# tulip-control/polytope

Hardware: AMD Instinct MI355X
Metric: LP solves/sec (batched Chebyshev + redundancy) (higher is better)
Workload: dtype f64

## Files before the change

polytope_amd/csrc/plp_lane_lp.hpp:

```cpp
#pragma once
#include <math.h>

#if defined(__HIPCC__)
#include "plp_common.hpp"
#define PLP_LANE_FN __device__ __forceinline__
#else
#define PLP_LANE_FN static inline
namespace plp {
enum : int { ST_OPT = 0, ST_ITER = 1, ST_INFEAS = 2, ST_UNBND = 3, ST_NUM = 4 };
constexpr int ST_RETRY = 5;
constexpr double TOL_D = 1e-9, TOL_PIV = 1e-7, DEGEN_EPS = 1e-12;
constexpr int BLAND_AFTER = 6;
}
#endif

namespace plp {
namespace lane {

constexpr int LANE_MAX_ITERS = 48;
constexpr double LANE_TOL_D = 1e-11, LANE_TOL_PIV = 1e-11;
constexpr double LANE_M_NOISE = 64 * 2.220446049250313e-16;

struct Lp3 {
    double x0, x1, x2;
    int w0, w1, w2;
    int nact;
    int status;
    int iters;
    int ndeg;
};

PLP_LANE_FN void cross3(double a0, double a1, double a2, double b0, double b1, double b2, double& e0, double& e1,
                        double& e2) {
    e0 = fma(a1, b2, -(a2 * b1));
    e1 = fma(a2, b0, -(a0 * b2));
    e2 = fma(a0, b1, -(a1 * b0));
}

PLP_LANE_FN double dot3(double a0, double a1, double a2, double b0, double b1, double b2) {
    return fma(a2, b2, fma(a1, b1, a0 * b0));
}

template <class AnyF>
PLP_LANE_FN void proj1(const double c0, const double c1, const double c2, const double cn1, const double n0, const double n1,
                       const double n2, const double nn, double& d0, double& d1, double& d2, double& scale, AnyF ANY) {
    const double cn = dot3(c0, c1, c2, n0, n1, n2);
    d0 = fma(cn, n0, -(nn * c0));
    d1 = fma(cn, n1, -(nn * c1));
    d2 = fma(cn, n2, -(nn * c2));
    scale = nn;
    const double pn1 = fabs(d0) + fabs(d1) + fabs(d2);
    const bool small = (pn1 > 0.0) & (pn1 < 1e-4 * (nn * cn1));
    if (ANY(small)) {
        const double np_ = dot3(n0, n1, n2, d0, d1, d2);
        const double q0 = fma(nn, d0, -(np_ * n0)), q1 = fma(nn, d1, -(np_ * n1)), q2 = fma(nn, d2, -(np_ * n2));
        d0 = small ? q0 : d0;
        d1 = small ? q1 : d1;
        d2 = small ? q2 : d2;
        scale = small ? nn * nn : nn;
    }
}

constexpr double LANE_PAIR_SIN2 = 1e-10;

template <class RowF, class RatioF, class Ratio0F, class AnyF>
PLP_LANE_FN void walk3(Lp3& S, const double c0, const double c1, const double c2, const bool go, RowF ROWS, RatioF RATIO,
                       Ratio0F RATIO0, AnyF ANY, const bool warm = false) {
    if (!warm) {
        S.x0 = S.x1 = S.x2 = 0.0;
        S.w0 = S.w1 = S.w2 = -1;
        S.nact = 0;
        S.iters = 0;
        S.ndeg = 0;
    }
    S.status = go ? -1 : ST_OPT;
    const double cn1 = fabs(c0) + fabs(c1) + fabs(c2);
    if (go && !(cn1 > 0.0)) S.status = ST_OPT;
    if (!warm && ANY(S.status < 0)) {
        const bool step = S.status < 0;
        const double d0 = -c0, d1 = -c1, d2 = -c2;
        const double tolp = LANE_TOL_PIV * cn1;
        double bs = 1.0, bd = 0.0;
        int bi = -1;
        RATIO0(d0, d1, d2, tolp, bs, bd, bi);
        if (step) {
            S.iters = 1;
            if (bi < 0) {
                S.status = ST_UNBND;
            } else {
                const double t = bs / bd;
                S.x0 = fma(t, d0, 0.0);
                S.x1 = fma(t, d1, 0.0);
                S.x2 = fma(t, d2, 0.0);
                S.w0 = bi;
                S.nact = 1;
                S.ndeg = (t * cn1 <= DEGEN_EPS) ? 1 : 0;
            }
        }
    }
    while (ANY(S.status < 0)) {
        const bool run = S.status < 0;
        double d0 = -c0, d1 = -c1, d2 = -c2;
        double n00 = 0, n01 = 0, n02 = 0, n10 = 0, n11 = 0, n12 = 0, n20 = 0, n21 = 0, n22 = 0;
        if (ANY(run && S.nact >= 1)) {
            if (S.nact >= 1) ROWS(S.w0, n00, n01, n02);
            if (S.nact >= 2) ROWS(S.w1, n10, n11, n12);
            if (S.nact >= 3) ROWS(S.w2, n20, n21, n22);
        }
        bool stalled = false;
        double dscale = cn1;
        if (S.nact == 1) {
            const double nn = dot3(n00, n01, n02, n00, n01, n02);
            double sc;
            proj1(c0, c1, c2, cn1, n00, n01, n02, nn, d0, d1, d2, sc, ANY);
            dscale = sc * cn1;
        } else if (S.nact == 2) {
            double e0, e1, e2;
            cross3(n00, n01, n02, n10, n11, n12, e0, e1, e2);
            const double ce = dot3(c0, c1, c2, e0, e1, e2);
            d0 = -(ce * e0);
            d1 = -(ce * e1);
            d2 = -(ce * e2);
            dscale = dot3(e0, e1, e2, e0, e1, e2) * cn1;
            const double nn0 = dot3(n00, n01, n02, n00, n01, n02), nn1 = dot3(n10, n11, n12, n10, n11, n12);
            if (run && !(dot3(e0, e1, e2, e0, e1, e2) > LANE_PAIR_SIN2 * nn0 * nn1)) S.status = ST_RETRY;
        } else if (S.nact == 3) {
            d0 = d1 = d2 = 0.0;
        }
        {
            const double dn1 = fabs(d0) + fabs(d1) + fabs(d2);
            stalled = !(dn1 > LANE_TOL_D * dscale);
        }
        if (ANY(S.status < 0 && stalled)) {
            if (S.status < 0 && stalled) {
                if (S.nact == 0) {
                    S.status = ST_OPT;
                } else if (S.nact == 1) {
                    const double cn = dot3(c0, c1, c2, n00, n01, n02);
                    if (cn <= 0.0) S.status = ST_OPT;
                    else { S.nact = 0; d0 = -c0; d1 = -c1; d2 = -c2; }
                } else if (S.nact == 2) {
                    const double g00 = dot3(n00, n01, n02, n00, n01, n02), g11 = dot3(n10, n11, n12, n10, n11, n12);
                    const double g01 = dot3(n00, n01, n02, n10, n11, n12);
                    const double r0 = -dot3(c0, c1, c2, n00, n01, n02), r1 = -dot3(c0, c1, c2, n10, n11, n12);
                    const double l0 = fma(r0, g11, -(r1 * g01)), l1 = fma(r1, g00, -(r0 * g01));
                    const double w0 = 0.5 * (1.0 + g00), w1 = 0.5 * (1.0 + g11);
                    const double tol0 = LANE_TOL_D * g11 * w0 * cn1, tol1 = LANE_TOL_D * g00 * w1 * cn1;
                    if (l0 >= -tol0 && l1 >= -tol1) S.status = ST_OPT;
                    else {
                        const bool drop0 = l0 * w0 < l1 * w1;
                        if (drop0) { S.w0 = S.w1; n00 = n10; n01 = n11; n02 = n12; }
                        S.nact = 1;
                        double sc;
                        proj1(c0, c1, c2, cn1, n00, n01, n02, dot3(n00, n01, n02, n00, n01, n02), d0, d1, d2, sc, [](bool q) { return q; });
                    }
                } else {
                    double u00, u01, u02, u10, u11, u12, u20, u21, u22;
                    cross3(n10, n11, n12, n20, n21, n22, u00, u01, u02);
                    cross3(n20, n21, n22, n00, n01, n02, u10, u11, u12);
                    cross3(n00, n01, n02, n10, n11, n12, u20, u21, u22);
                    const double det = dot3(n00, n01, n02, u00, u01, u02);
                    const double g00 = dot3(n00, n01, n02, n00, n01, n02), g11 = dot3(n10, n11, n12, n10, n11, n12);
                    const double g22 = dot3(n20, n21, n22, n20, n21, n22);
                    if (!(det * det > 1e-18 * (g00 * g11 * g22))) {
                        S.status = ST_RETRY;
                    } else {
                        const double sg = det > 0.0 ? 1.0 : -1.0;
                        const double l0 = -sg * dot3(c0, c1, c2, u00, u01, u02);
                        const double l1 = -sg * dot3(c0, c1, c2, u10, u11, u12);
                        const double l2 = -sg * dot3(c0, c1, c2, u20, u21, u22);
                        const double a0 = l0 * (0.5 * (1.0 + g00)), a1 = l1 * (0.5 * (1.0 + g11)), a2 = l2 * (0.5 * (1.0 + g22));
                        const double tol = LANE_TOL_D * fabs(det) * cn1;
                        if (a0 >= -tol && a1 >= -tol && a2 >= -tol) S.status = ST_OPT;
                        else {
                            int j = 0;
                            double am = a0;
                            if (a1 < am) { am = a1; j = 1; }
                            if (a2 < am) { am = a2; j = 2; }
                            double gg;
                            if (j == 0) { d0 = -sg * u00; d1 = -sg * u01; d2 = -sg * u02; S.w0 = S.w1; S.w1 = S.w2; gg = g11 * g22; }
                            else if (j == 1) { d0 = -sg * u10; d1 = -sg * u11; d2 = -sg * u12; S.w1 = S.w2; gg = g22 * g00; }
                            else { d0 = -sg * u20; d1 = -sg * u21; d2 = -sg * u22; gg = g00 * g11; }
                            S.nact = 2;
                            if (!(dot3(d0, d1, d2, d0, d1, d2) > LANE_PAIR_SIN2 * gg)) S.status = ST_RETRY;
                        }
                    }
                }
            }
        }
        const bool step = S.status < 0;
        const double dn1 = fabs(d0) + fabs(d1) + fabs(d2);
        const double tolp = LANE_TOL_PIV * dn1;
        double bs = 1.0, bd = 0.0;
        int bi = -1;
        if (ANY(step)) RATIO(d0, d1, d2, S.x0, S.x1, S.x2, tolp, bs, bd, bi);
        if (step) {
            ++S.iters;
            if (bi < 0) {
                S.status = ST_UNBND;
            } else {
                const double t = bs / bd;
                S.x0 = fma(t, d0, S.x0);
                S.x1 = fma(t, d1, S.x1);
                S.x2 = fma(t, d2, S.x2);
                if (S.nact == 0) S.w0 = bi;
                else if (S.nact == 1) S.w1 = bi;
                else S.w2 = bi;
                S.nact += 1;
                S.ndeg = (t * dn1 <= DEGEN_EPS) ? S.ndeg + 1 : 0;
                if (S.ndeg >= BLAND_AFTER || S.iters >= LANE_MAX_ITERS) S.status = ST_RETRY;
            }
        }
    }
}

template <class RowF, class RatioF, class AnyF>
PLP_LANE_FN void walk3(Lp3& S, const double c0, const double c1, const double c2, const bool go, RowF ROWS, RatioF RATIO,
                       AnyF ANY, const bool warm = false) {
    walk3(S, c0, c1, c2, go, ROWS, RATIO,
          [&](double d0, double d1, double d2, double tolp, double& bs, double& bd, int& bi) {
              RATIO(d0, d1, d2, 0.0, 0.0, 0.0, tolp, bs, bd, bi);
          },
          ANY, warm);
}

struct Lp4 {
    double x0, x1, x2, x3;
    int w0, w1, w2, w3;
    int nact, status, iters, ndeg;
};

PLP_LANE_FN double dot4(double a0, double a1, double a2, double a3, double b0, double b1, double b2, double b3) {
    return fma(a3, b3, fma(a2, b2, fma(a1, b1, a0 * b0)));
}

PLP_LANE_FN void gcross4(double p0, double p1, double p2, double p3, double q0, double q1, double q2, double q3, double r0,
                         double r1, double r2, double r3, double& e0, double& e1, double& e2, double& e3) {
    const double m01 = fma(q0, r1, -(q1 * r0)), m02 = fma(q0, r2, -(q2 * r0)), m03 = fma(q0, r3, -(q3 * r0));
    const double m12 = fma(q1, r2, -(q2 * r1)), m13 = fma(q1, r3, -(q3 * r1)), m23 = fma(q2, r3, -(q3 * r2));
    e0 = fma(p1, m23, fma(-p2, m13, p3 * m12));
    e1 = -fma(p0, m23, fma(-p2, m03, p3 * m02));
    e2 = fma(p0, m13, fma(-p1, m03, p3 * m01));
    e3 = -fma(p0, m12, fma(-p1, m02, p2 * m01));
}

template <class RowF, class RatioF, class AnyF>
PLP_LANE_FN void walk4(Lp4& S, const double c0, const double c1, const double c2, const double c3, const bool go, RowF ROWS,
                       RatioF RATIO, AnyF ANY) {
    S.x0 = S.x1 = S.x2 = S.x3 = 0.0;
    S.w0 = S.w1 = S.w2 = S.w3 = -1;
    S.nact = 0;
    S.iters = 0;
    S.ndeg = 0;
    S.status = go ? -1 : ST_OPT;
    const double cn1 = fabs(c0) + fabs(c1) + fabs(c2) + fabs(c3);
    if (go && !(cn1 > 0.0)) S.status = ST_OPT;
    while (ANY(S.status < 0)) {
        const bool run = S.status < 0;
        bool dropped = false;
        double d0 = -c0, d1 = -c1, d2 = -c2, d3 = -c3;
        double n00 = 0, n01 = 0, n02 = 0, n03 = 0, n10 = 0, n11 = 0, n12 = 0, n13 = 0;
        double n20 = 0, n21 = 0, n22 = 0, n23 = 0, n30 = 0, n31 = 0, n32 = 0, n33 = 0;
        if (ANY(run && S.nact >= 1)) {
            if (S.nact >= 1) ROWS(S.w0, n00, n01, n02, n03);
            if (S.nact >= 2) ROWS(S.w1, n10, n11, n12, n13);
            if (S.nact >= 3) ROWS(S.w2, n20, n21, n22, n23);
            if (S.nact >= 4) ROWS(S.w3, n30, n31, n32, n33);
        }
        const double g00 = dot4(n00, n01, n02, n03, n00, n01, n02, n03), g11 = dot4(n10, n11, n12, n13, n10, n11, n12, n13);
        const double g22 = dot4(n20, n21, n22, n23, n20, n21, n22, n23);
        const double g01 = dot4(n00, n01, n02, n03, n10, n11, n12, n13), g02 = dot4(n00, n01, n02, n03, n20, n21, n22, n23);
        const double g12 = dot4(n10, n11, n12, n13, n20, n21, n22, n23);
        const double r0 = dot4(c0, c1, c2, c3, n00, n01, n02, n03), r1 = dot4(c0, c1, c2, c3, n10, n11, n12, n13);
        const double r2 = dot4(c0, c1, c2, c3, n20, n21, n22, n23);
        double det = 1.0, m0 = 0.0, m1 = 0.0, m2 = 0.0;
        if (S.nact == 1) {
            det = g00;
            m0 = r0;
        } else if (S.nact == 2) {
            det = fma(g00, g11, -(g01 * g01));
            m0 = fma(r0, g11, -(r1 * g01));
            m1 = fma(r1, g00, -(r0 * g01));
            if (run && !(det > LANE_PAIR_SIN2 * g00 * g11)) S.status = ST_RETRY;
        } else if (S.nact == 3) {
            const double A00 = fma(g11, g22, -(g12 * g12)), A01 = fma(g02, g12, -(g01 * g22)), A02 = fma(g01, g12, -(g02 * g11));
            const double A11 = fma(g00, g22, -(g02 * g02)), A12 = fma(g01, g02, -(g00 * g12)), A22 = fma(g00, g11, -(g01 * g01));
            det = fma(g00, A00, fma(g01, A01, g02 * A02));
            m0 = fma(A00, r0, fma(A01, r1, A02 * r2));
            m1 = fma(A01, r0, fma(A11, r1, A12 * r2));
            m2 = fma(A02, r0, fma(A12, r1, A22 * r2));
            if (run && !(det > 1e-16 * g00 * g11 * g22)) S.status = ST_RETRY;
        }
        bool twice = false;
        if (S.nact == 3) {
            double e0, e1, e2, e3;
            gcross4(n00, n01, n02, n03, n10, n11, n12, n13, n20, n21, n22, n23, e0, e1, e2, e3);
            const double ce = dot4(c0, c1, c2, c3, e0, e1, e2, e3);
            d0 = -(ce * e0);
            d1 = -(ce * e1);
            d2 = -(ce * e2);
            d3 = -(ce * e3);
        } else if (S.nact >= 1 && S.nact <= 2) {
            d0 = fma(m1, n10, fma(m0, n00, -(det * c0)));
            d1 = fma(m1, n11, fma(m0, n01, -(det * c1)));
            d2 = fma(m1, n12, fma(m0, n02, -(det * c2)));
            d3 = fma(m1, n13, fma(m0, n03, -(det * c3)));
            if (S.nact == 1) {
                const double nd = dot4(n00, n01, n02, n03, d0, d1, d2, d3);
                d0 = fma(g00, d0, -(nd * n00));
                d1 = fma(g00, d1, -(nd * n01));
                d2 = fma(g00, d2, -(nd * n02));
                d3 = fma(g00, d3, -(nd * n03));
            } else {
                const double dn = fabs(d0) + fabs(d1) + fabs(d2) + fabs(d3);
                twice = (dn > 0.0) & (dn < 1e-4 * (det * cn1));
                if (ANY(run && twice)) {
                    const double s0 = dot4(d0, d1, d2, d3, n00, n01, n02, n03), s1 = dot4(d0, d1, d2, d3, n10, n11, n12, n13);
                    const double k0 = fma(s0, g11, -(s1 * g01)), k1 = fma(s1, g00, -(s0 * g01));
                    const double q0 = fma(det, d0, -fma(k1, n10, k0 * n00)), q1 = fma(det, d1, -fma(k1, n11, k0 * n01));
                    const double q2 = fma(det, d2, -fma(k1, n12, k0 * n02)), q3 = fma(det, d3, -fma(k1, n13, k0 * n03));
                    d0 = twice ? q0 : d0;
                    d1 = twice ? q1 : d1;
                    d2 = twice ? q2 : d2;
                    d3 = twice ? q3 : d3;
                }
            }
        } else if (S.nact == 4) {
            d0 = d1 = d2 = d3 = 0.0;
        }
        const double dscale = (S.nact >= 1 && S.nact <= 3) ? ((S.nact == 1 || twice) ? det * det : det) * cn1 : cn1;
        const bool stalled = !(fabs(d0) + fabs(d1) + fabs(d2) + fabs(d3) > LANE_TOL_D * dscale);
        if (ANY(S.status < 0 && stalled)) {
            if (S.status < 0 && stalled) {
                const double w0 = 0.5 * (1.0 + g00), w1 = 0.5 * (1.0 + g11), w2 = 0.5 * (1.0 + g22);
                if (S.nact == 0) {
                    S.status = ST_OPT;
                } else if (S.nact <= 3) {
                    const double tol = LANE_TOL_D * det * cn1;
                    double f0 = 0.0, f1 = 0.0, f2 = 0.0;
                    if (S.nact == 2) {
                        f0 = fabs(r0 * g11) + fabs(r1 * g01);
                        f1 = fabs(r1 * g00) + fabs(r0 * g01);
                    } else if (S.nact == 3) {
                        const double B00 = fabs(g11 * g22) + g12 * g12, B01 = fabs(g02 * g12) + fabs(g01 * g22), B02 = fabs(g01 * g12) + fabs(g02 * g11);
                        const double B11 = fabs(g00 * g22) + g02 * g02, B12 = fabs(g01 * g02) + fabs(g00 * g12), B22 = fabs(g00 * g11) + g01 * g01;
                        f0 = B00 * fabs(r0) + B01 * fabs(r1) + B02 * fabs(r2);
                        f1 = B01 * fabs(r0) + B11 * fabs(r1) + B12 * fabs(r2);
                        f2 = B02 * fabs(r0) + B12 * fabs(r1) + B22 * fabs(r2);
                    }
                    const double a0 = -m0 * w0, a1 = S.nact >= 2 ? -m1 * w1 : 0.0, a2 = S.nact >= 3 ? -m2 * w2 : 0.0;
                    const double t0 = fmax(tol, LANE_M_NOISE * f0 * w0), t1 = fmax(tol, LANE_M_NOISE * f1 * w1), t2 = fmax(tol, LANE_M_NOISE * f2 * w2);
                    if (a0 >= -t0 && a1 >= -t1 && a2 >= -t2) {
                        S.status = ST_OPT;
                    } else {
                        int j = 0;
                        double am = a0 + t0;
                        if (a1 + t1 < am) { am = a1 + t1; j = 1; }
                        if (a2 + t2 < am) { am = a2 + t2; j = 2; }
                        if (j == 0) S.w0 = S.w1;
                        if (j <= 1) S.w1 = S.w2;
                        S.nact -= 1;
                        dropped = true;
                    }
                } else {
                    const double g33 = dot4(n30, n31, n32, n33, n30, n31, n32, n33);
                    const double w3 = 0.5 * (1.0 + g33);
                    double am = 0.0, bd0 = 0.0, bd1 = 0.0, bd2 = 0.0, bd3 = 0.0, dj_abs = 0.0;
                    int jbest = -1;
                    bool all_ok = true, singular = false;
#define PLP_W4_VERTEX(J, P, Q, R, NJ0, NJ1, NJ2, NJ3, WJ)                                                          \
                    {                                                                                                   \
                        double u0, u1, u2, u3;                                                                          \
                        gcross4(P##0, P##1, P##2, P##3, Q##0, Q##1, Q##2, Q##3, R##0, R##1, R##2, R##3, u0, u1, u2, u3); \
                        const double dj = dot4(NJ0, NJ1, NJ2, NJ3, u0, u1, u2, u3);                                     \
                        const double sg = dj > 0.0 ? 1.0 : -1.0;                                                        \
                        const double lj = -sg * dot4(c0, c1, c2, c3, u0, u1, u2, u3);                                   \
                        const double aj = lj * (WJ);                                                                    \
                        dj_abs = fabs(dj);                                                                              \
                        singular = singular | !(dj * dj > 1e-18 * (g00 * g11 * g22 * g33));                            \
                        all_ok = all_ok & (aj >= -(LANE_TOL_D * dj_abs * cn1));                                              \
                        const bool better = (jbest < 0) | (aj < am);                                                    \
                        am = better ? aj : am;                                                                          \
                        jbest = better ? (J) : jbest;                                                                   \
                        bd0 = better ? -sg * u0 : bd0;                                                                  \
                        bd1 = better ? -sg * u1 : bd1;                                                                  \
                        bd2 = better ? -sg * u2 : bd2;                                                                  \
                        bd3 = better ? -sg * u3 : bd3;                                                                  \
                    }
                    PLP_W4_VERTEX(0, n1, n2, n3, n00, n01, n02, n03, w0)
                    PLP_W4_VERTEX(1, n0, n2, n3, n10, n11, n12, n13, w1)
                    PLP_W4_VERTEX(2, n0, n1, n3, n20, n21, n22, n23, w2)
                    PLP_W4_VERTEX(3, n0, n1, n2, n30, n31, n32, n33, w3)
#undef PLP_W4_VERTEX
                    if (singular) S.status = ST_RETRY;
                    else if (all_ok) S.status = ST_OPT;
                    else {
                        d0 = bd0; d1 = bd1; d2 = bd2; d3 = bd3;
                        if (jbest == 0) S.w0 = S.w1;
                        if (jbest <= 1) S.w1 = S.w2;
                        if (jbest <= 2) S.w2 = S.w3;
                        S.nact = 3;
                    }
                }
            }
        }
        if (dropped) {
            ++S.iters;
            if (S.iters >= LANE_MAX_ITERS) S.status = ST_RETRY;
        }
        const bool step = (S.status < 0) & !dropped;
        const double dn1 = fabs(d0) + fabs(d1) + fabs(d2) + fabs(d3);
        const double tolp = LANE_TOL_PIV * dn1;
        double bs = 1.0, bd = 0.0;
        int bi = -1;
        if (ANY(step)) RATIO(d0, d1, d2, d3, S.x0, S.x1, S.x2, S.x3, tolp, bs, bd, bi);
        if (step) {
            ++S.iters;
            if (bi < 0) {
                S.status = ST_UNBND;
            } else {
                const double t = bs / bd;
                S.x0 = fma(t, d0, S.x0);
                S.x1 = fma(t, d1, S.x1);
                S.x2 = fma(t, d2, S.x2);
                S.x3 = fma(t, d3, S.x3);
                if (S.nact == 0) S.w0 = bi;
                else if (S.nact == 1) S.w1 = bi;
                else if (S.nact == 2) S.w2 = bi;
                else S.w3 = bi;
                S.nact += 1;
                S.ndeg = (t * dn1 <= DEGEN_EPS) ? S.ndeg + 1 : 0;
                if (S.ndeg >= BLAND_AFTER || S.iters >= LANE_MAX_ITERS) S.status = ST_RETRY;
            }
        }
    }
}

PLP_LANE_FN void ratio_row4(const double a0, const double a1, const double a2, const double a3, const double beta, const int i,
                            const double d0, const double d1, const double d2, const double d3, const double x0,
                            const double x1, const double x2, const double x3, const double tolp, double& bs, double& bd,
                            int& bi) {
    const double ad = dot4(a0, a1, a2, a3, d0, d1, d2, d3);
    const double ax = dot4(a0, a1, a2, a3, x0, x1, x2, x3);
    const double sl = fmax(beta - ax, 0.0);
    const bool better = (ad > tolp) & (sl * bd < bs * ad);
    bs = better ? sl : bs;
    bd = better ? ad : bd;
    bi = better ? i : bi;
}

PLP_LANE_FN void ratio_row(const double a0, const double a1, const double a2, const double beta, const int i, const double d0,
                           const double d1, const double d2, const double x0, const double x1, const double x2,
                           const double tolp, double& bs, double& bd, int& bi) {
    const double ad = dot3(a0, a1, a2, d0, d1, d2);
    const double ax = dot3(a0, a1, a2, x0, x1, x2);
    const double sl = fmax(beta - ax, 0.0);
    const bool better = (ad > tolp) & (sl * bd < bs * ad);
    bs = better ? sl : bs;
    bd = better ? ad : bd;
    bi = better ? i : bi;
}

PLP_LANE_FN void ratio_row0(const double a0, const double a1, const double a2, const double beta, const int i, const double d0,
                            const double d1, const double d2, const double tolp, double& bs, double& bd, int& bi) {
    const double ad = dot3(a0, a1, a2, d0, d1, d2);
    const double sl = fmax(beta, 0.0);
    const bool better = (ad > tolp) & (sl * bd < bs * ad);
    bs = better ? sl : bs;
    bd = better ? ad : bd;
    bi = better ? i : bi;
}

template <int M, class RowF, class BetaF, class AnyF, class PassF>
PLP_LANE_FN void solve3(Lp3& S, const double c0, const double c1, const double c2, const bool go, RowF ROWS, BetaF BETA,
                        AnyF ANY, PassF PASS, const bool warm = false) {
    walk3(S, c0, c1, c2, go, ROWS,
          [&](double d0, double d1, double d2, double x0, double x1, double x2, double tolp, double& bs, double& bd, int& bi) {
              PASS();
#pragma unroll
              for (int i = 0; i < M; ++i) {
                  double a0, a1, a2;
                  ROWS(i, a0, a1, a2);
                  ratio_row(a0, a1, a2, BETA(i), i, d0, d1, d2, x0, x1, x2, tolp, bs, bd, bi);
              }
          },
          ANY, warm);
}

template <int M, class RowF, class BetaF, class AnyF>
PLP_LANE_FN void solve3(Lp3& S, const double c0, const double c1, const double c2, const bool go, RowF ROWS, BetaF BETA,
                        AnyF ANY, const bool warm = false) {
    solve3<M>(S, c0, c1, c2, go, ROWS, BETA, ANY, [] {}, warm);
}

}
}
```

polytope_amd/csrc/plp_reduce_lane.hpp:

```cpp
#pragma once
#include <type_traits>

#include "plp_lane_lp.hpp"
#include "plp_reduce_general.hpp"
#include "plp_reduce_r_impl.hpp"

namespace plp {

#ifndef PLP_LANE_CH
#define PLP_LANE_CH 4
#endif

constexpr int LN_ROWS = 16;

template <int D, int GS, int ROWS>
__device__ __noinline__ void reduce_lane_redo(unsigned char* smem_raw, const long long tile, const int ntile, const uint64_t rb64,
                                              int m_max, const double* __restrict__ Ag, const double* __restrict__ bg,
                                              const int* __restrict__ mrows, double abs_tol,
                                              unsigned long long* __restrict__ keep_out, int* __restrict__ flags_out,
                                              double* __restrict__ r_out, double* __restrict__ xc_out,
                                              int* __restrict__ nlp_out) {
    constexpr int PER = 64 / ROWS;
    for (int sub = 0; sub < (64 / GS) / PER; ++sub) {
        unsigned some = 0u;
#pragma unroll
        for (int q = 0; q < PER; ++q) some |= (unsigned)((rb64 >> (GS * (PER * sub + q))) & 1ull) << q;
        if (some == 0u) continue;
        const int q = (threadIdx.x & 63) / ROWS;
        const bool mine = ((some >> q) & 1u) != 0u;
        const int left = ntile - PER * sub;
        reduce_general_tile<D, RBLOCK>(smem_raw, tile + PER * sub, left < PER ? left : PER, mine, m_max, ROWS, Ag, bg, mrows, abs_tol,
                                       keep_out, flags_out, r_out, xc_out, nlp_out);
    }
}

template <int D, int GS, int ROWS = LN_ROWS, bool BBOX = false>
__device__ __forceinline__ void reduce_lane_tile(
    const long long tile, long long B, int m_max, const double* __restrict__ Ag, const double* __restrict__ bg,
    const int* __restrict__ mrows, double abs_tol, int force_retry, unsigned long long* __restrict__ keep_out,
    int* __restrict__ flags_out, double* __restrict__ r_out, double* __restrict__ xc_out, int* __restrict__ nlp_out,
    unsigned long long* __restrict__ ctr) {
    static_assert(D >= 1 && D <= 4, "the lane engine walks in R^3 (lower dimensions are embedded) or R^4");
    static_assert(RBLOCK == 64, "one wavefront per workgroup");
    static_assert(GS == 4 || GS == 8 || GS == 16, "lanes per polytope");
    static_assert((ROWS == 16 || ROWS == 32) && ROWS / GS >= 1 && ROWS / GS <= 4, "row slots per polytope, at most four per lane");
    constexpr int rows = ROWS, R = rows / GS, NG = 64 / GS;
    constexpr unsigned RMASK = (1u << R) - 1u;
    constexpr int LS = NG;
    extern __shared__ __attribute__((aligned(16))) unsigned char smem_raw[];
    const Grp g(GS);
    const int lane = g.lane;
    const int gib = lane / GS;
    const int row0 = g.gl * R;
    double* sA = reinterpret_cast<double*>(smem_raw);
    double* sb = sA + (size_t)rows * D * NG;
    double* san = sb + (size_t)rows * NG;
    double* myA = sA + gib;
    constexpr int OFF_B = rows * D * NG, OFF_N = OFF_B + rows * NG;
    double* const myb = myA + OFF_B;
    double* const myan = myA + OFF_N;
#define LA(i, kk) myA[((i) * D + (kk)) * LS]
#define LB(i) myA[OFF_B + (i) * LS]
#define LN(i) myA[OFF_N + (i) * LS]
    double* const rA = myA + row0 * D * LS;
    double* const rS = myA + row0 * LS;
#define OA(k, kk) rA[((k) * D + (kk)) * LS]
#define OB(k) rS[OFF_B + (k) * LS]
#define ON(k) rS[OFF_N + (k) * LS]
    const double qnan = __longlong_as_double(0x7ff8000000000000ll);
    const double pinf = __longlong_as_double(0x7ff0000000000000ll);
    const int ntile = (B - tile) < NG ? (int)(B - tile) : NG;
    __syncthreads();
    {
        const int p = lane % NG, q = lane / NG;
        const int rowsz = m_max * D;
        const bool pv = p < ntile;
        const double* src = Ag + (tile + (pv ? p : 0)) * rowsz;
        double va[rows * D / GS], vb[rows / GS];
        const double* srcb = bg + (tile + (pv ? p : 0)) * m_max;
        if (m_max == rows) {
#pragma unroll
            for (int it = 0; it < rows * D / GS; ++it) va[it] = src[q + GS * it];
#pragma unroll
            for (int it = 0; it < rows / GS; ++it) vb[it] = srcb[q + GS * it];
        } else {
#pragma unroll
            for (int it = 0; it < rows * D / GS; ++it) {
                const int rem = q + GS * it;
                va[it] = src[rem < rowsz ? rem : 0];
            }
#pragma unroll
            for (int it = 0; it < rows / GS; ++it) {
                const int row = q + GS * it;
                vb[it] = srcb[row < m_max ? row : 0];
            }
        }
#pragma unroll
        for (int it = 0; it < rows * D / GS; ++it) {
            const int rem = q + GS * it;
            sA[rem * NG + p] = (pv & (rem < rowsz)) ? va[it] : 0.0;
        }
#pragma unroll
        for (int it = 0; it < rows / GS; ++it) {
            const int row = q + GS * it;
            sb[row * NG + p] = (pv & (row < m_max)) ? vb[it] : 0.0;
        }
    }
    __syncthreads();
    const bool valid = gib < ntile;
    const int m = valid ? (mrows ? (mrows + tile)[gib] : m_max) : 0;
    double xc[D];
    double rr = 0.0;
    bool ball, fulldim, f1open = false;
    uint64_t live = 0ull;
    unsigned has = 0u;
    bool retry = force_retry != 0;
    {
        SimplexR<D + 1, R, false, true> S;
        double qi[R];
        S.reset(D + 1, m, row0);
        unsigned actb = 0u;
        bool inf0 = false, finite = true;
#pragma unroll
        for (int k = 0; k < R; ++k) {
            const bool h = valid & (row0 + k < m) & (m <= rows);
            has |= h ? (1u << k) : 0u;
            double nrm2 = 0.0;
#pragma unroll
            for (int kk = 0; kk < D; ++kk) {
                const double v = h ? OA(k, kk) : 0.0;
                S.T[k][kk] = v;
                nrm2 = nrm2 + v * v;
                finite = finite & isfinite(v);
            }
            const double bk = h ? OB(k) : 0.0;
            finite = finite & isfinite(bk);
            const double nrm = sqrt(nrm2);
            ON(k) = 1.0 / nrm;
            const bool zero = !(nrm > 0.0);
            const bool on = h & !zero;
            S.T[k][D] = on ? nrm : 0.0;
            S.beta[k] = on ? bk : 0.0;
            qi[k] = bk / nrm;
            actb |= on ? (1u << k) : 0u;
            inf0 = inf0 | (h & zero & (bk < -TOL_FEAS));
        }
        S.ract = actb;
        const bool infeasible0 = grp_ballot(inf0, g) != 0;
        const bool bad = (grp_ballot(!finite, g) != 0) | (m > rows);
        S.cost[D] = -1.0;
        S.mode = M_P2;
        if (!valid | bad) { S.mode = M_DONE; S.status = ST_NUM; }
        else if (infeasible0) { S.mode = M_DONE; S.status = ST_INFEAS; }
#ifndef PLP_LANE_DBG_NOF1
        S.template run_fast<GS, true>(g, qi, actb);
#endif
        retry = retry | (valid & (S.status == ST_RETRY));
        const bool ok = S.status == ST_OPT;
        f1open = valid & !ok & (S.status != ST_INFEAS);
#pragma unroll
        for (int j = 0; j <= D; ++j) {
            bool found;
            const double mine = S.x_of(j, found);
            const uint64_t ob = grp_ballot(found, g);
            const double v = bcast(mine, g.gbase + (ob ? __ffsll((long long)ob) - 1 : 0));
            const double xj = ob ? v : 0.0;
            if (j < D) xc[j < D ? j : 0] = xj; else rr = xj;
        }
        ball = ok & (rr >= 0.0);
        fulldim = ball & (rr > abs_tol);
        if constexpr (BBOX) fulldim = ball & (rr >= 1e-6);
    }
    if (!BBOX && (valid & (g.gl == 0))) {
        (r_out + tile)[gib] = ball ? rr : 0.0;
#pragma unroll
        for (int k = 0; k < D; ++k) (xc_out + tile * D)[gib * D + k] = ball ? xc[k] : qnan;
    }
    __syncthreads();
#ifdef PLP_LANE_DBG_F1ONLY
    if (valid & (g.gl == 0)) { (keep_out + tile)[gib] = 0; (flags_out + tile)[gib] = 0; (nlp_out + tile)[gib] = 1; }
    return;
#endif
    if constexpr (BBOX) {
#pragma unroll
        for (int k = 0; k < R; ++k) live |= spread_rows<R, GS>(grp_ballot(((has >> k) & 1u) != 0u, g)) << k;
    } else {
        unsigned remmask = 0u;
        const double scr_thr = sqrt(2.0 * abs_tol) * 1.0001 + 1e-12;
        double ni[R][D], bin_[R];
#pragma unroll
        for (int k = 0; k < R; ++k) {
            const double an_i = ON(k);
#pragma unroll
            for (int kk = 0; kk < D; ++kk) ni[k][kk] = OA(k, kk) * an_i;
            bin_[k] = OB(k) * an_i;
        }
#pragma unroll 2
        for (int t = 1; t <= rows / 2; ++t) {
#pragma unroll
            for (int k = 0; k < R; ++k) {
                const int i = row0 + k;
                const int j = (i + t) & (rows - 1);
                const double an_j = LN(j);
                if (!__any(fabs(ni[k][0] - LA(j, 0) * an_j) < scr_thr)) continue;
                double dot = 0.0;
#pragma unroll
                for (int kk = 0; kk < D; ++kk) dot = dot + ni[k][kk] * (LA(j, kk) * an_j);
                const double bjn = LB(j) * an_j;
                const bool par = valid & (m <= rows) & (i < m) & (j < m) & (dot > 1.0 - abs_tol);
                const bool i_lo = i < j;
                const double blo = i_lo ? bin_[k] : bjn, bhi = i_lo ? bjn : bin_[k];
                const int lo = i_lo ? i : j, hi = i_lo ? j : i;
                const int gone = (blo < bhi) ? hi : lo;
                remmask |= par ? (1u << gone) : 0u;
            }
        }
#pragma unroll
        for (int o = 1; o < GS; o <<= 1) remmask |= (unsigned)__shfl_xor((int)remmask, o, 64);
        const unsigned removed = (remmask >> row0) & RMASK;
#pragma unroll
        for (int k = 0; k < R; ++k)
            live |= spread_rows<R, GS>(grp_ballot((((has & ~removed) >> k) & 1u) != 0u, g)) << k;
    }
    bool neg = false;
#pragma unroll
    for (int k = 0; k < R; ++k) {
        double sk = 0.0;
#pragma unroll
        for (int kk = 0; kk < D; ++kk) sk = fma(((has >> k) & 1u) ? OA(k, kk) : 0.0, ball ? xc[kk] : 0.0, sk);
        const double raw = (((has >> k) & 1u) ? OB(k) : 0.0) - sk;
        neg = neg | (raw < 0.0);
        ON(k) = fmax(raw, 0.0);
    }
    if (__any(neg & ball)) {
        bool off = false;
        const double xs = centre_scale<D>(xc);
#pragma unroll
        for (int k = 0; k < R; ++k) {
            const bool hk = ((has >> k) & 1u) != 0u;
            double sk = 0.0, nrm2 = 0.0;
#pragma unroll
            for (int kk = 0; kk < D; ++kk) {
                const double v = hk ? OA(k, kk) : 0.0;
                sk = fma(v, ball ? xc[kk] : 0.0, sk);
                nrm2 = nrm2 + v * v;
            }
            const double bk = hk ? OB(k) : 0.0;
            off = off | (hk & centre_off(bk - sk, 1.0 / sqrt(nrm2), bk, xs));
        }
        if (ball & (grp_ballot(off, g) != 0)) {
            ball = false; fulldim = false; f1open = true;
            if (!BBOX && (valid & (g.gl == 0))) {
                (r_out + tile)[gib] = 0.0;
#pragma unroll
                for (int k = 0; k < D; ++k) (xc_out + tile * D)[gib * D + k] = qnan;
            }
        }
    }
    auto zero_dead = [&](unsigned alive) {
#pragma unroll
        for (int k = 0; k < R; ++k) {
            if (!((alive >> k) & 1u)) {
#pragma unroll
                for (int kk = 0; kk < D; ++kk) OA(k, kk) = 0.0;
                OB(k) = 0.0;
                ON(k) = 0.0;
            }
        }
    };
    zero_dead(((unsigned)(live >> row0) & RMASK));
    int flags = fulldim ? 0 : (RF_EMPTY | (f1open ? RF_F1OPEN : 0));
    int nlp = 1;
    uint64_t keep = 0ull;
    int stage = 0;
    if (fulldim) {
        const int neq = __popcll(live);
        if (neq <= D + 1) { flags = RF_EARLY; keep = live; }
        else stage = (neq > 3 * D) ? 1 : 2;
        if constexpr (BBOX) stage = 1;
    }
    __syncthreads();
    auto any_lane = [](bool p) { return __any(p) != 0; };
    using LpState = std::conditional_t<D == 4, lane::Lp4, lane::Lp3>;
    auto lane_solve = [&](LpState& S, const double (&cv)[4], const bool go_, const double* pA, const double* pbeta, auto relax_tag,
                          int krv, const int nparts, const int part) {
        constexpr bool RELAX = decltype(relax_tag)::value;
        const int cnt = rows / nparts;
        const int i0 = part * cnt;
        auto row_of = [&](const double* base, double& a0, double& a1, double& a2, double& a3) {
            a0 = base[0];
            a1 = D > 1 ? base[(D > 1 ? 1 : 0) * LS] : 0.0;
            a2 = D > 2 ? base[(D > 2 ? 2 : 0) * LS] : 0.0;
            a3 = D > 3 ? base[(D > 3 ? 3 : 0) * LS] : 0.0;
        };
        auto ratio = [&](auto x0_tag, const double (&dv)[4], const double (&xv)[4], double tolp, double& bs, double& bd, int& bi) {
            constexpr bool X0 = decltype(x0_tag)::value;
            if constexpr (RELAX) asm volatile("" : "+v"(krv));
            const double* ra = pA + i0 * D * LS;
            const double* rb_ = pbeta + i0 * LS;
            int ic = i0;
            for (int ch = 0; ch < cnt; ch += PLP_LANE_CH) {
#pragma unroll
                for (int r = 0; r < PLP_LANE_CH; ++r) {
                    double a0, a1, a2, a3;
                    row_of(ra + (r * D) * LS, a0, a1, a2, a3);
                    double beta = rb_[r * LS];
                    if constexpr (RELAX) beta = beta + ((ic + r == krv) ? 0.1 : 0.0);
                    if constexpr (D == 4)
                        lane::ratio_row4(a0, a1, a2, a3, beta, ic + r, dv[0], dv[1], dv[2], dv[3], xv[0], xv[1], xv[2], xv[3], tolp,
                                         bs, bd, bi);
                    else if constexpr (X0)
                        lane::ratio_row0(a0, a1, a2, beta, ic + r, dv[0], dv[1], dv[2], tolp, bs, bd, bi);
                    else
                        lane::ratio_row(a0, a1, a2, beta, ic + r, dv[0], dv[1], dv[2], xv[0], xv[1], xv[2], tolp, bs, bd, bi);
                }
                ra += PLP_LANE_CH * D * LS;
                rb_ += PLP_LANE_CH * LS;
                ic += PLP_LANE_CH;
            }
            auto meet = [&](auto ctrl) {
                constexpr int CTRL = decltype(ctrl)::value;
                const double ps = dpp_d<CTRL>(bs), pd = dpp_d<CTRL>(bd);
                const int pi = dpp_i<CTRL>(bi);
                const double l = ps * bd, r_ = bs * pd;
                const bool theirs = (pd > 0.0) & (!(bd > 0.0) | (l < r_) | ((l == r_) & (pi < bi)));
                bs = theirs ? ps : bs;
                bd = theirs ? pd : bd;
                bi = theirs ? pi : bi;
            };
            if (nparts > 1) meet(std::integral_constant<int, PLP_DPP_XOR1>{});
            if (nparts > 2) meet(std::integral_constant<int, PLP_DPP_XOR2>{});
        };
        if constexpr (D == 4) {
            lane::walk4(
                S, cv[0], cv[1], cv[2], cv[3], go_,
                [&](int i, double& a0, double& a1, double& a2, double& a3) { row_of(pA + (i * D) * LS, a0, a1, a2, a3); },
                [&](double d0, double d1, double d2, double d3, double x0, double x1, double x2, double x3, double tolp, double& bs,
                    double& bd, int& bi) {
                    const double dv[4] = {d0, d1, d2, d3}, xv[4] = {x0, x1, x2, x3};
                    ratio(std::false_type{}, dv, xv, tolp, bs, bd, bi);
                },
                any_lane);
        } else {
            lane::walk3(
                S, cv[0], cv[1], cv[2], go_,
                [&](int i, double& a0, double& a1, double& a2) {
                    double a3;
                    row_of(pA + (i * D) * LS, a0, a1, a2, a3);
                },
                [&](double d0, double d1, double d2, double x0, double x1, double x2, double tolp, double& bs, double& bd, int& bi) {
                    const double dv[4] = {d0, d1, d2, 0.0}, xv[4] = {x0, x1, x2, 0.0};
                    ratio(std::false_type{}, dv, xv, tolp, bs, bd, bi);
                },
                [&](double d0, double d1, double d2, double tolp, double& bs, double& bd, int& bi) {
                    const double dv[4] = {d0, d1, d2, 0.0}, xv[4] = {0.0, 0.0, 0.0, 0.0};
                    ratio(std::true_type{}, dv, xv, tolp, bs, bd, bi);
                },
                any_lane);
        }
    };
    auto x_of_lp = [](const LpState& S, int k) {
        double v = k == 0 ? S.x0 : (k == 1 ? S.x1 : S.x2);
        if constexpr (D == 4) v = k == 3 ? S.x3 : v;
        return v;
    };
#ifdef PLP_LANE_DBG_NOF3
    if (false) {
#else
    if (__any(stage == 1)) {
#endif
        const bool go = stage == 1;
        const unsigned lloc = ((unsigned)(live >> row0) & RMASK);
        bool lpfail = false;
        constexpr int NLP = 2 * D;
        constexpr int NROUND = GS == 16 ? 1 : (NLP + GS - 1) / GS;
        auto f3_pair = [](int rd) { return GS == 16 || 2 * (NLP - rd * GS < GS ? NLP - rd * GS : GS) <= GS; };
        auto f3_round_of = [](int it) { return GS == 16 ? 0 : it / GS; };
        auto f3_lane_of = [&](int it) { const int rd = f3_round_of(it); return f3_pair(rd) ? 2 * (it - rd * GS) : it - rd * GS; };
        double val[NROUND];
#pragma unroll
        for (int q = 0; q < NROUND; ++q) val[q] = 0.0;
#pragma unroll 1
        for (int rd = 0; rd < NROUND; ++rd) {
            const bool pair = f3_pair(rd);
            const int nparts = pair ? 2 : 1;
            const int it = rd * GS + (pair ? (g.gl >> 1) : g.gl);
            const int part = pair ? (g.gl & 1) : 0;
            const bool mine = go & (it < 2 * D);
            const int kx = it >> 1;
            const bool up = it & 1;
            const double cs = up ? -1.0 : 1.0;
            LpState S;
            const double cv[4] = {kx == 0 ? cs : 0.0, kx == 1 ? cs : 0.0, kx == 2 ? cs : 0.0, kx == 3 ? cs : 0.0};
            lane_solve(S, cv, mine, myA, myan, std::false_type{}, -1, nparts, part);
            double xck = 0.0;
#pragma unroll
            for (int kk = 0; kk < D; ++kk) xck = (kk == kx) ? xc[kk] : xck;
            const double xk = x_of_lp(S, kx);
            double v;
            if (S.status == ST_OPT) v = xck + xk;
            else if (S.status == ST_UNBND) v = up ? pinf : -pinf;
            else { v = qnan; lpfail = lpfail | (mine & (S.status != ST_RETRY)); }
            retry = retry | (mine & (S.status == ST_RETRY));
            if constexpr (BBOX) {
                double* xfin = reinterpret_cast<double*>(keep_out);
                if (xfin && (valid & mine & (part == 0))) {
#pragma unroll
                    for (int kk = 0; kk < D; ++kk) xfin[((size_t)(tile + gib) * 2 * D + it) * D + kk] = xc[kk] + x_of_lp(S, kk);
                }
            }
#pragma unroll
            for (int q = 0; q < NROUND; ++q) val[q] = (q == rd) ? v : val[q];
        }
        lpfail = grp_ballot(lpfail, g) != 0;
        retry = retry | (grp_ballot(retry, g) != 0);
        if constexpr (BBOX) {
#pragma unroll
            for (int it2 = 0; it2 < NLP; ++it2) {
                const double v = bcast(val[f3_round_of(it2)], g.gbase + f3_lane_of(it2));
                if (valid & (g.gl == 0)) ((it2 & 1) ? xc_out + tile * D : r_out + tile * D)[gib * D + (it2 >> 1)] = go ? v : qnan;
            }
            if (valid & (g.gl == 0)) (flags_out + tile)[gib] = (go & !retry & !lpfail) ? 0 : 1;
            return;
        }
        double s1[R], s2[R];
#pragma unroll
        for (int k = 0; k < R; ++k) { s1[k] = 0.0; s2[k] = 0.0; }
#pragma unroll
        for (int kx = 0; kx < D; ++kx) {
            const int itl = 2 * kx, ith = 2 * kx + 1;
            const double lo = bcast(val[f3_round_of(itl)], g.gbase + f3_lane_of(itl));
            const double hi = bcast(val[f3_round_of(ith)], g.gbase + f3_lane_of(ith));
#pragma unroll
            for (int k = 0; k < R; ++k) {
                const double aik = OA(k, kx);
                const double pa = (aik > 0.0 ? 1.0 : 0.0) * aik;
                s1[k] = s1[k] + pa * (hi - lo);
                s2[k] = s2[k] + aik * lo;
            }
        }
        uint64_t outb = 0ull;
#pragma unroll
        for (int k = 0; k < R; ++k) {
            const bool out = go & (((lloc >> k) & 1u) != 0u) & ((s1[k] - (OB(k) - s2[k])) < -1e-4);
            outb |= spread_rows<R, GS>(grp_ballot(out, g)) << k;
        }
        __syncthreads();
        if (go) {
            live = live & ~outb;
            zero_dead(((unsigned)(live >> row0) & RMASK));
            nlp += 2 * D;
            if (lpfail) flags |= RF_LPFAIL;
            if (__popcll(live) <= D + 1) { flags |= RF_EARLY; keep = live; stage = 0; }
            else stage = 2;
        }
        __syncthreads();
    }
    if constexpr (BBOX) {
        if (valid & (g.gl == 0)) {
            (flags_out + tile)[gib] = 1;
#pragma unroll
            for (int k = 0; k < D; ++k) { (r_out + tile * D)[gib * D + k] = qnan; (xc_out + tile * D)[gib * D + k] = qnan; }
        }
        return;
    }
#ifdef PLP_LANE_DBG_NOF2
    if (false) {
#else
    if (__any(stage == 2)) {
#endif
        const unsigned lloc = ((unsigned)(live >> row0) & RMASK);
        uint64_t todo = (stage == 2) ? live : 0ull;
        if (stage == 2) nlp += __popcll(live);
#ifndef PLP_LANE_DBG_NOPRE
        {
            const unsigned okb = f2_presolve<D, R, LS, true>(myA, myb, myan, row0, m_max, (stage == 2) ? lloc : 0u, abs_tol);
            uint64_t cert = 0ull;
#pragma unroll
            for (int k = 0; k < R; ++k) cert |= spread_rows<R, GS>(grp_ballot(((okb >> k) & 1u) != 0u, g)) << k;
            keep |= cert;
            todo &= ~cert;
            ctr_add(ctr, -__popcll(cert), g.gl == 0);
        }
#endif
        __syncthreads();
        const unsigned todo32 = (unsigned)todo;
        const int n_g = __popc(todo32);
        int total = 0, nmax = 0;
        for (int p = 0; p < NG; ++p) {
            const int np = __builtin_amdgcn_readlane(n_g, p * GS);
            total += np;
            nmax = np > nmax ? np : nmax;
        }
        int off_g = 0;
        for (int p = 0, run = 0; p < NG; ++p) {
            off_g = (gib == p) ? run : off_g;
            run += __builtin_amdgcn_readlane(n_g, p * GS);
        }
        unsigned retry_polys = 0u;
        int rb = 0;
        while (rb < total) {
            const int nrem = total - rb;
            const int nparts = nrem <= 16 ? 4 : (nrem <= 32 ? 2 : 1);
            const int sh = nparts == 4 ? 2 : (nparts == 2 ? 1 : 0);
            const int per = 64 >> sh;
            const int t = rb + (lane >> sh);
            const int part = lane & (nparts - 1);
            int tp = 0, toff = 0, run = 0;
            unsigned ttd = 0u;
            for (int p = 0; p < NG; ++p) {
                const int np = __builtin_amdgcn_readlane(n_g, p * GS);
                const unsigned tdp = (unsigned)__builtin_amdgcn_readlane((int)todo32, p * GS);
                const bool at = t >= run;
                tp = at ? p : tp;
                ttd = at ? tdp : ttd;
                toff = at ? run : toff;
                run += np;
            }
            const bool mine = t < total;
            {
                const int rank = t - toff;
                for (int i = 0; i < nmax; ++i) ttd = (i < rank) ? (ttd & (ttd - 1u)) : ttd;
            }
            const int kr = mine ? (__ffs((int)ttd) - 1) : 0;
            const double* pA = sA + tp;
            const double* pan = pA + OFF_N;
            double c[4] = {0.0, 0.0, 0.0, 0.0};
#pragma unroll
            for (int kk = 0; kk < D; ++kk) c[kk] = -pA[(kr * D + kk) * LS];
            LpState S;
            lane_solve(S, c, mine, pA, pan, std::true_type{}, kr, nparts, part);
            double akx = -lane::dot3(c[0], c[1], c[2], S.x0, S.x1, S.x2);
            if constexpr (D == 4) akx = -lane::dot4(c[0], c[1], c[2], c[3], S.x0, S.x1, S.x2, S.x3);
            const double obj = akx - pan[kr * LS];
            const bool keepk = mine & (((S.status == ST_OPT) & (obj > abs_tol)) | (S.status == ST_UNBND));
            const uint64_t all = __ballot(keepk);
            const uint64_t rt = __ballot(mine & (S.status == ST_RETRY));
            if (rt != 0ull) {
                for (int p = 0; p < NG; ++p)
                    if (__any(mine & (S.status == ST_RETRY) & (tp == p))) retry_polys |= 1u << p;
            }
#pragma unroll
            for (int k = 0; k < R; ++k) {
                const int rw = row0 + k;
                const int tt = off_g + __popc(todo32 & ((1u << rw) - 1u)) - rb;
                const bool own = (((todo32 >> rw) & 1u) != 0u) & (tt >= 0) & (tt < per);
                const bool kept = own & (((all >> ((tt << sh) & 63)) & 1ull) != 0ull);
                keep |= spread_rows<R, GS>(grp_ballot(kept, g)) << k;
            }
            rb += per;
        }
        retry = retry | (((retry_polys >> gib) & 1u) != 0u);
        if (stage == 2) flags |= RF_MINREP;
    }
    if (valid & (g.gl == 0) & !retry) {
        (keep_out + tile)[gib] = keep;
        (flags_out + tile)[gib] = flags;
        (nlp_out + tile)[gib] = nlp;
    }
    ctr_add(ctr, nlp, valid & (g.gl == 0));
    const uint64_t rb64 = __ballot(retry & valid & (g.gl == 0));
    if (rb64 != 0ull) {
        __threadfence_block();
        __syncthreads();
        reduce_lane_redo<D, GS, ROWS>(smem_raw, tile, ntile, rb64, m_max, Ag, bg, mrows, abs_tol, keep_out, flags_out, r_out, xc_out,
                            nlp_out);
    }
#undef LA
#undef OA
#undef OB
#undef ON
#undef LB
#undef LN
}

#ifndef PLP_REDUCE_LANE_WAVES
#define PLP_REDUCE_LANE_WAVES(D) ((D) <= 3 ? 4 : 3)
#endif

template <int D, int GS, int ROWS = LN_ROWS>
__global__ __launch_bounds__(RBLOCK, PLP_REDUCE_LANE_WAVES(D)) void reduce_lane_kernel(
    long long B, int m_max, const double* __restrict__ Ag, const double* __restrict__ bg, const int* __restrict__ mrows,
    double abs_tol, int force_retry, unsigned long long* __restrict__ keep_out, int* __restrict__ flags_out,
    double* __restrict__ r_out, double* __restrict__ xc_out, int* __restrict__ nlp_out, unsigned long long* __restrict__ ctr) {
    reduce_lane_tile<D, GS, ROWS>((long long)blockIdx.x * (64 / GS), B, m_max, Ag, bg, mrows, abs_tol, force_retry, keep_out,
                                  flags_out, r_out, xc_out, nlp_out, ctr);
}

template <int D, int ROWS, int GSA, int GSB>
__global__ __launch_bounds__(RBLOCK, PLP_REDUCE_LANE_WAVES(D)) void reduce_lane_mix_kernel(
    int nbig, long long B, int m_max, const double* __restrict__ Ag, const double* __restrict__ bg,
    const int* __restrict__ mrows, double abs_tol, int force_retry, unsigned long long* __restrict__ keep_out,
    int* __restrict__ flags_out, double* __restrict__ r_out, double* __restrict__ xc_out, int* __restrict__ nlp_out,
    unsigned long long* __restrict__ ctr) {
    constexpr int NA = 64 / GSA, NB_ = 64 / GSB;
    if ((int)blockIdx.x < nbig)
        reduce_lane_tile<D, GSA, ROWS>((long long)blockIdx.x * NA, B, m_max, Ag, bg, mrows, abs_tol, force_retry, keep_out,
                                       flags_out, r_out, xc_out, nlp_out, ctr);
    else
        reduce_lane_tile<D, GSB, ROWS>((long long)nbig * NA + (long long)((int)blockIdx.x - nbig) * NB_, B, m_max, Ag, bg, mrows,
                                       abs_tol, force_retry, keep_out, flags_out, r_out, xc_out, nlp_out, ctr);
}

template <int D, int GS, int ROWS>
__global__ __launch_bounds__(RBLOCK, PLP_REDUCE_LANE_WAVES(D)) void bbox_lane_kernel(
    long long B, int m_max, const double* __restrict__ Ag, const double* __restrict__ bg, const int* __restrict__ mrows,
    int force_retry, double* __restrict__ lb, double* __restrict__ ub, int* __restrict__ status, double* __restrict__ xfin) {
    reduce_lane_tile<D, GS, ROWS, true>((long long)blockIdx.x * (64 / GS), B, m_max, Ag, bg, mrows, 0.0, force_retry,
                                        reinterpret_cast<unsigned long long*>(xfin), status, lb, ub, nullptr, nullptr);
}

}
```

Baseline: 13.38 billion.

## Factor lane ratio test into exec-masked latch with axis-aligned first pass

Result: faster. 14.15 billion (median of 6 runs) (+5.7%).

```diff
diff --git a/polytope_amd/csrc/plp_lane_lp.hpp b/polytope_amd/csrc/plp_lane_lp.hpp
--- a/polytope_amd/csrc/plp_lane_lp.hpp
+++ b/polytope_amd/csrc/plp_lane_lp.hpp
@@ -471,6 +471,89 @@
     bi = better ? i : bi;
 }
 
+#ifndef PLP_LANE_CH
+#define PLP_LANE_CH 4
+#endif
+
+PLP_LANE_FN void latch_row(const bool elig, const bool closer, const double sl, const double ad, const int i, double& bs,
+                           double& bd, int& bi) {
+#if defined(__HIP_DEVICE_COMPILE__) && !defined(PLP_LANE_SELECT_LATCH)
+    const unsigned long long mask = __builtin_amdgcn_ballot_w64(elig) & __builtin_amdgcn_ballot_w64(closer);
+    unsigned long long saved;
+    asm("s_and_saveexec_b64 %[sv], %[m]\n\t"
+        "v_mov_b64 %[bs], %[sl]\n\t"
+        "v_mov_b64 %[bd], %[ad]\n\t"
+        "v_mov_b32 %[bi], %[i]\n\t"
+        "s_mov_b64 exec, %[sv]"
+        : [bs] "+v"(bs), [bd] "+v"(bd), [bi] "+v"(bi), [sv] "=&s"(saved)
+        : [m] "s"(mask), [sl] "v"(sl), [ad] "v"(ad), [i] "s"(i)
+        : "scc");
+#else
+    const bool better = elig & closer;
+    bs = better ? sl : bs;
+    bd = better ? ad : bd;
+    bi = better ? i : bi;
+#endif
+}
+
+PLP_LANE_FN double relax_row(const bool at, double beta) {
+#if defined(__HIP_DEVICE_COMPILE__) && !defined(PLP_LANE_SELECT_LATCH)
+    const unsigned long long mask = __builtin_amdgcn_ballot_w64(at);
+    unsigned long long saved;
+    asm("s_and_saveexec_b64 %[sv], %[m]\n\t"
+        "v_add_f64 %[b], %[b], %[c]\n\t"
+        "s_mov_b64 exec, %[sv]"
+        : [b] "+v"(beta), [sv] "=&s"(saved)
+        : [m] "s"(mask), [c] "s"(0.1)
+        : "scc");
+    return beta;
+#else
+    return at ? beta + 0.1 : beta;
+#endif
+}
+
+enum : int { RATIO_WALK = 0, RATIO_FIRST = 1, RATIO_AXIS = 2 };
+
+template <int D, int LS, int MODE, bool RELAX>
+PLP_LANE_FN void ratio_rows(const double* pA, const double* pbeta, const int i0, const int cnt, const int krv,
+                            const double (&dv)[4], const double (&xv)[4], const int kax, const double dk, const double tolp,
+                            double& bs, double& bd, int& bi) {
+    static_assert(D >= 1 && D <= 4 && (D < 4 || MODE == RATIO_WALK), "R^4 has no peeled first pass");
+    const double* ra = pA + i0 * D * LS + (MODE == RATIO_AXIS ? kax * LS : 0);
+    const double* rb = pbeta + i0 * LS;
+    const int krel = krv - i0;
+    int li = -1;
+    for (int ch = 0; ch < cnt; ch += PLP_LANE_CH) {
+#pragma unroll
+        for (int r = 0; r < PLP_LANE_CH; ++r) {
+            const double* a = ra + (r * D) * LS;
+            double beta = rb[r * LS];
+            if constexpr (RELAX) beta = relax_row(ch + r == krel, beta);
+            double ad, sl;
+            if constexpr (MODE == RATIO_AXIS) {
+                ad = dk * a[0];
+                sl = fmax(beta, 0.0);
+            } else {
+                const double a0 = a[0];
+                const double a1 = D > 1 ? a[(D > 1 ? 1 : 0) * LS] : 0.0;
+                const double a2 = D > 2 ? a[(D > 2 ? 2 : 0) * LS] : 0.0;
+                if constexpr (D == 4) {
+                    const double a3 = a[(D > 3 ? 3 : 0) * LS];
+                    ad = dot4(a0, a1, a2, a3, dv[0], dv[1], dv[2], dv[3]);
+                    sl = fmax(fma(-a3, xv[3], fma(-a2, xv[2], fma(-a1, xv[1], fma(-a0, xv[0], beta)))), 0.0);
+                } else {
+                    ad = dot3(a0, a1, a2, dv[0], dv[1], dv[2]);
+                    sl = MODE == RATIO_FIRST ? fmax(beta, 0.0) : fmax(fma(-a2, xv[2], fma(-a1, xv[1], fma(-a0, xv[0], beta))), 0.0);
+                }
+            }
+            latch_row(ad > tolp, sl * bd < bs * ad, sl, ad, ch + r, bs, bd, li);
+        }
+        ra += PLP_LANE_CH * D * LS;
+        rb += PLP_LANE_CH * LS;
+    }
+    bi = li < 0 ? bi : li + i0;
+}
+
 template <int M, class RowF, class BetaF, class AnyF, class PassF>
 PLP_LANE_FN void solve3(Lp3& S, const double c0, const double c1, const double c2, const bool go, RowF ROWS, BetaF BETA,
                         AnyF ANY, PassF PASS, const bool warm = false) {
diff --git a/polytope_amd/csrc/plp_reduce_lane.hpp b/polytope_amd/csrc/plp_reduce_lane.hpp
--- a/polytope_amd/csrc/plp_reduce_lane.hpp
+++ b/polytope_amd/csrc/plp_reduce_lane.hpp
@@ -6,10 +6,6 @@
 #include "plp_reduce_r_impl.hpp"
 
 namespace plp {
-
-#ifndef PLP_LANE_CH
-#define PLP_LANE_CH 4
-#endif
 
 constexpr int LN_ROWS = 16;
 
@@ -270,7 +266,7 @@
     };
     zero_dead(((unsigned)(live >> row0) & RMASK));
     int flags = fulldim ? 0 : (RF_EMPTY | (f1open ? RF_F1OPEN : 0));
-    int nlp = 1;
+    int nlp = 1, presolved = 0;
     uint64_t keep = 0ull;
     int stage = 0;
     if (fulldim) {
@@ -283,8 +279,9 @@
     auto any_lane = [](bool p) { return __any(p) != 0; };
     using LpState = std::conditional_t<D == 4, lane::Lp4, lane::Lp3>;
     auto lane_solve = [&](LpState& S, const double (&cv)[4], const bool go_, const double* pA, const double* pbeta, auto relax_tag,
-                          int krv, const int nparts, const int part) {
+                          int krv, const int nparts, const int part, const int kax, const double dk) {
         constexpr bool RELAX = decltype(relax_tag)::value;
+        constexpr int FIRST = RELAX ? lane::RATIO_FIRST : lane::RATIO_AXIS;
         const int cnt = rows / nparts;
         const int i0 = part * cnt;
         auto row_of = [&](const double* base, double& a0, double& a1, double& a2, double& a3) {
@@ -293,31 +290,10 @@
             a2 = D > 2 ? base[(D > 2 ? 2 : 0) * LS] : 0.0;
             a3 = D > 3 ? base[(D > 3 ? 3 : 0) * LS] : 0.0;
         };
-        auto ratio = [&](auto x0_tag, const double (&dv)[4], const double (&xv)[4], double tolp, double& bs, double& bd, int& bi) {
-            constexpr bool X0 = decltype(x0_tag)::value;
+        auto ratio = [&](auto mode_tag, const double (&dv)[4], const double (&xv)[4], double tolp, double& bs, double& bd, int& bi) {
+            constexpr int MODE = decltype(mode_tag)::value;
             if constexpr (RELAX) asm volatile("" : "+v"(krv));
-            const double* ra = pA + i0 * D * LS;
-            const double* rb_ = pbeta + i0 * LS;
-            int ic = i0;
-            for (int ch = 0; ch < cnt; ch += PLP_LANE_CH) {
-#pragma unroll
-                for (int r = 0; r < PLP_LANE_CH; ++r) {
-                    double a0, a1, a2, a3;
-                    row_of(ra + (r * D) * LS, a0, a1, a2, a3);
-                    double beta = rb_[r * LS];
-                    if constexpr (RELAX) beta = beta + ((ic + r == krv) ? 0.1 : 0.0);
-                    if constexpr (D == 4)
-                        lane::ratio_row4(a0, a1, a2, a3, beta, ic + r, dv[0], dv[1], dv[2], dv[3], xv[0], xv[1], xv[2], xv[3], tolp,
-                                         bs, bd, bi);
-                    else if constexpr (X0)
-                        lane::ratio_row0(a0, a1, a2, beta, ic + r, dv[0], dv[1], dv[2], tolp, bs, bd, bi);
-                    else
-                        lane::ratio_row(a0, a1, a2, beta, ic + r, dv[0], dv[1], dv[2], xv[0], xv[1], xv[2], tolp, bs, bd, bi);
-                }
-                ra += PLP_LANE_CH * D * LS;
-                rb_ += PLP_LANE_CH * LS;
-                ic += PLP_LANE_CH;
-            }
+            lane::ratio_rows<D, LS, MODE, RELAX>(pA, pbeta, i0, cnt, krv, dv, xv, kax, dk, tolp, bs, bd, bi);
             auto meet = [&](auto ctrl) {
                 constexpr int CTRL = decltype(ctrl)::value;
                 const double ps = dpp_d<CTRL>(bs), pd = dpp_d<CTRL>(bd);
@@ -338,7 +314,7 @@
                 [&](double d0, double d1, double d2, double d3, double x0, double x1, double x2, double x3, double tolp, double& bs,
                     double& bd, int& bi) {
                     const double dv[4] = {d0, d1, d2, d3}, xv[4] = {x0, x1, x2, x3};
-                    ratio(std::false_type{}, dv, xv, tolp, bs, bd, bi);
+                    ratio(std::integral_constant<int, lane::RATIO_WALK>{}, dv, xv, tolp, bs, bd, bi);
                 },
                 any_lane);
         } else {
@@ -350,11 +326,11 @@
                 },
                 [&](double d0, double d1, double d2, double x0, double x1, double x2, double tolp, double& bs, double& bd, int& bi) {
                     const double dv[4] = {d0, d1, d2, 0.0}, xv[4] = {x0, x1, x2, 0.0};
-                    ratio(std::false_type{}, dv, xv, tolp, bs, bd, bi);
+                    ratio(std::integral_constant<int, lane::RATIO_WALK>{}, dv, xv, tolp, bs, bd, bi);
                 },
                 [&](double d0, double d1, double d2, double tolp, double& bs, double& bd, int& bi) {
                     const double dv[4] = {d0, d1, d2, 0.0}, xv[4] = {0.0, 0.0, 0.0, 0.0};
-                    ratio(std::true_type{}, dv, xv, tolp, bs, bd, bi);
+                    ratio(std::integral_constant<int, FIRST>{}, dv, xv, tolp, bs, bd, bi);
                 },
                 any_lane);
         }
@@ -392,7 +368,7 @@
             const double cs = up ? -1.0 : 1.0;
             LpState S;
             const double cv[4] = {kx == 0 ? cs : 0.0, kx == 1 ? cs : 0.0, kx == 2 ? cs : 0.0, kx == 3 ? cs : 0.0};
-            lane_solve(S, cv, mine, myA, myan, std::false_type{}, -1, nparts, part);
+            lane_solve(S, cv, mine, myA, myan, std::false_type{}, -1, nparts, part, kx < D ? kx : 0, up ? 1.0 : -1.0);
             double xck = 0.0;
 #pragma unroll
             for (int kk = 0; kk < D; ++kk) xck = (kk == kx) ? xc[kk] : xck;
@@ -480,7 +456,7 @@
             for (int k = 0; k < R; ++k) cert |= spread_rows<R, GS>(grp_ballot(((okb >> k) & 1u) != 0u, g)) << k;
             keep |= cert;
             todo &= ~cert;
-            ctr_add(ctr, -__popcll(cert), g.gl == 0);
+            presolved = __popcll(cert);
         }
 #endif
         __syncthreads();
@@ -529,7 +505,7 @@
 #pragma unroll
             for (int kk = 0; kk < D; ++kk) c[kk] = -pA[(kr * D + kk) * LS];
             LpState S;
-            lane_solve(S, c, mine, pA, pan, std::true_type{}, kr, nparts, part);
+            lane_solve(S, c, mine, pA, pan, std::true_type{}, kr, nparts, part, 0, 0.0);
             double akx = -lane::dot3(c[0], c[1], c[2], S.x0, S.x1, S.x2);
             if constexpr (D == 4) akx = -lane::dot4(c[0], c[1], c[2], c[3], S.x0, S.x1, S.x2, S.x3);
             const double obj = akx - pan[kr * LS];
@@ -558,7 +534,7 @@
         (flags_out + tile)[gib] = flags;
         (nlp_out + tile)[gib] = nlp;
     }
-    ctr_add(ctr, nlp, valid & (g.gl == 0));
+    ctr_add(ctr, nlp - presolved, valid & (g.gl == 0));
     const uint64_t rb64 = __ballot(retry & valid & (g.gl == 0));
     if (rb64 != 0ull) {
         __threadfence_block();
```
